# Dellintel98/smart-nanogrid-gym

Hardware: AMD Instinct MI355X
Metric: env-steps/sec (whole node) at N=65,536 envs × 10 chargers, 24-step day (higher is better)
Workload: dtype f64; 1 GPU; 65536 envs/GPU x 10 chargers x 24-step day, b-pv bounded sparse 1h, GPU-RNG reset + 24 fused steps per bench step (hipGraph); envs_per_gpu=65536, chargers=10, step_unit=one simulated day of every env, days_per_graph_replay=11, parallelism=env-sharded x1

## Files before the change

smart-nanogrid-gym_amd/csrc/sng_dev_env.h:

```cpp
#pragma once

namespace sng {

__device__ __forceinline__ void write_obs_header(float *o, const Params &p, const double *irr, const double *pn,
                                                 double ratio, const double *fpv, const double *fpr) {
    int k = 0;
    if (p.pv) o[k++] = (float)((irr[0] * ratio) * fpv[0]);
    o[k++] = (float)(pn[0] * fpr[0]);
    if (p.pv) {
#pragma unroll
        for (int j = 1; j <= 3; ++j) o[k++] = (float)((irr[j] * ratio) * fpv[j]);
    }
#pragma unroll
    for (int j = 1; j <= 3; ++j) o[k++] = (float)(pn[j] * fpr[j]);
}

__device__ __forceinline__ void write_obs_header_station(float *o, const double *irr, const float *pnf, double ratio) {
    o[0] = (float)(irr[0] * ratio);
    o[1] = pnf[0];
#pragma unroll
    for (int j = 1; j <= 3; ++j) {
        o[1 + j] = (float)(irr[j] * ratio);
        o[4 + j] = pnf[j];
    }
}

__device__ __forceinline__ uint32_t mix32(uint32_t x) {
    x ^= x >> 17;
    x *= 0xed5ad4bbu;
    x ^= x >> 11;
    x *= 0xac4c1b51u;
    x ^= x >> 15;
    x *= 0x31848babu;
    x ^= x >> 14;
    return x;
}

__device__ __forceinline__ uint32_t stream_key(uint64_t seed, uint64_t ge, uint32_t lane, uint64_t day) {
    const uint32_t k0 = mix32((uint32_t)seed ^ mix32((uint32_t)(seed >> 32) + (uint32_t)day * 0x9e3779b9u));
    const uint32_t k1 = mix32(k0 ^ (uint32_t)ge);
    return mix32(k1 ^ ((uint32_t)(ge >> 32) * 0x85ebca6bu + lane * 0xc2b2ae35u + 0x27d4eb2fu));
}

constexpr uint32_t kDomainPV = 0x50560000u;
constexpr uint32_t kDomainPrice = 0x50520000u;

__device__ __forceinline__ double profile_factor_key(uint32_t key, int k, double sigma) {
    if (sigma == 0.0) return 1.0;
    const uint32_t h = mix32(key + (uint32_t)k * 0x9e3779b9u);
    const double z = (double)h * 0x1.0p-31 - 1.0;
    return 1.0 + sigma * z;
}
__device__ __forceinline__ double profile_factor(uint64_t env_seed, uint32_t domain, uint64_t day, int k,
                                                 double sigma) {
    return profile_factor_key(stream_key(env_seed, 0, domain, day), k, sigma);
}
__device__ __forceinline__ v2u profile_keys(const DeviceState &s, uint32_t el8) {
    return __builtin_bit_cast(v2u, bld(reinterpret_cast<const uint64_t *>(s.prof_key), el8));
}
__device__ __forceinline__ void expand_profile_factors(const Params &p, v2u kk, int t, double *fpv, double *fpr) {
#pragma unroll
    for (int j = 0; j < 4; ++j) {
        fpv[j] = profile_factor_key(kk.x, t + j, p.pv_noise);
        fpr[j] = profile_factor_key(kk.y, t + j, p.price_noise);
    }
}
__device__ __forceinline__ void profile_factors(const Params &p, const DeviceState &s, uint32_t el8, int t,
                                                double *fpv, double *fpr) {
    expand_profile_factors(p, profile_keys(s, el8), t, fpv, fpr);
}

enum { CST_IRR = 0, CST_PN = 4, CST_PV = 8, CST_PRICE = 9, CST_COUNT = 10 };
__host__ __device__ inline double step_constant(const Tables *tb, int t, int i) {
    return i < CST_PN ? tb->irr_norm[t + i]
                      : i < CST_PV ? tb->price_norm[t + i - CST_PN] : i == CST_PV ? tb->pv_power[t] : tb->price[t];
}

__device__ __forceinline__ double step_constant_scalar(const Tables *tb, int t, int i) {
    typedef const __attribute__((address_space(4))) double *ConstF64;
    const double *q = i < CST_PN ? &tb->irr_norm[t + i]
                                 : i < CST_PV ? &tb->price_norm[t + i - CST_PN] : i == CST_PV ? &tb->pv_power[t] : &tb->price[t];
    return *(ConstF64)(uintptr_t)q;
}

template <bool PK = false>
__device__ __forceinline__ float departure_obs(uint32_t w) {
    const float d = PK ? (float)(w >> P_DEP_SHIFT) : (float)((w >> W_DEP_SHIFT) & 0xffu);
    constexpr float r24 = 1.0f / 24.0f;
    const float q = d * r24;
    return __builtin_fmaf(__builtin_fmaf(-q, 24.0f, d), r24, q);
}

__device__ __forceinline__ double div_by_cap(double x, double c, double r) {
    const double q = x * r;
    return __builtin_fma(__builtin_fmin(__builtin_fma(-q, c, x), q), r, q);
}

__device__ __forceinline__ double recip_cap(double c) {
    const double r0 = __builtin_amdgcn_rcp(c);
    return __builtin_fma(r0, __builtin_fma(-c, r0, 1.0), r0);
}

struct ChargerResult {
    double pw;
    double q;
    double soc;
    uint32_t nx;
    uint32_t fl;
};

template <bool FAST, bool NONNEG = false, bool PK = false>
__device__ __forceinline__ ChargerResult charger_step(const Params &p, uint32_t w, double aux, double run, double req,
                                                      float a, int t, double rcap) {
    ChargerResult o;
    SNG_DIAG_CHARGER(o, aux, run, a);
    const double margin = 0.05 * req;
    const double d = (req - run) * 10;
    const bool insufficient = (t > 0) && (w & W_PEN) && (run < req - margin);
    o.q = insufficient ? d * d : 0.0;

    const bool occ = (w & W_OCC) != 0;
    const double prev = (occ && !(w & W_STATIC)) ? run : aux;
    const uint32_t capi = cap_field<PK>(w);
    const double cap = (double)capi;
    const bool idle = (a == 0.0f);
    const bool chg = (a > 0.0f);
    static_assert(FAST || !NONNEG, "the NONNEG form is the wide kernel's: NumPy-2 promotion");
    double pc, calc, calc_dis;
    float pf = 0.0f;
    if (!FAST && p.legacy) {
        pc = ((double)a * p.ev_power) * p.ev_eff;
        calc = calc_dis = prev + (pc * p.dt) / cap;
    } else {
        pf = __fmul_rn(__fmul_rn(a, p.ev_power_f), p.ev_eff_f);
        const float pdt = __fmul_rn(pf, p.dt_f);
        pc = (double)pf;
        const double mag = div_by_cap(NONNEG ? (double)pdt : __builtin_fabs((double)pdt), cap, rcap);
        calc = prev + mag;
        calc_dis = prev - mag;
    }
    if constexpr (NONNEG) {
        const bool moved = occ && chg && p.bounded;
        o.soc = moved ? ((1.0 < calc) ? 1.0 : calc) : prev;
        o.pw = (double)(moved ? pf : 0.0f);
        o.nx = (!occ && chg) ? 1u : 0u;
        o.fl = (occ && chg && !p.bounded) ? (uint32_t)SNG_FLAG_CHARGING_MODE : 0u;
        return o;
    }
    double pw_dis = pc;
    if (FAST) {
        pw_dis = !(calc_dis < 0.0) ? -((prev * cap) * p.rdt) : pc;
    } else if (occ && !idle && !chg && !(calc_dis < 0.0)) {
        const double x = prev * cap;
        pw_dis = -(p.dt_pow2 ? x * p.rdt : x / p.dt);
    }
    const double soc_chg = (1.0 < calc) ? 1.0 : calc;
    const double soc_dis = (calc_dis > 0.0) ? calc_dis : 0.0;
    const bool moved = occ && !idle && p.bounded;
    o.soc = moved ? (chg ? soc_chg : soc_dis) : prev;
    o.pw = moved ? (chg ? pc : pw_dis) : 0.0;
    o.nx = (!occ && !idle) ? 1u : 0u;
    o.fl = (occ && !idle && !p.bounded) ? (uint32_t)SNG_FLAG_CHARGING_MODE : 0u;
    return o;
}

template <bool PK>
struct ChargerVisit {
    ChargerResult r;
    double soc;
    uint32_t w_dep;
    __device__ __forceinline__ float obs_soc() const { return (float)r.soc; }
    __device__ __forceinline__ float obs_dep() const { return departure_obs<PK>(w_dep); }
};
template <bool FAST, bool NONNEG, bool PK, bool TABLE = false>
__device__ __forceinline__ ChargerVisit<PK> visit_charger(const Params &p, uint32_t w, const double &aux, double run,
                                                          double req, float a, int t, const double *rcp_table = nullptr) {
    const uint32_t capi = cap_field<PK>(w);
    const bool occ = (w & W_OCC) != 0;
    ChargerVisit<PK> v{charger_step<FAST, NONNEG, PK>(p, PK ? (w & ~W_STATIC) : w, PK ? 0.0 : aux, run, req, a, t,
                                                      TABLE ? rcp_table[capi] : recip_cap((double)capi)),
                       0.0, (PK && !occ) ? 0u : w};
    v.soc = (PK && !occ) ? (double)rec_soc(w) : v.r.soc;
    return v;
}

struct BessStep {
    double bess, pen_b, bpow, bcalc, pw, dp;
    bool moved, chg;
    uint32_t fl;
};
template <bool STORE = true>
__device__ __forceinline__ BessStep bess_step(const Params &p, const DeviceState &s, uint32_t el8, int t, double bess,
                                              float bess_action) {
    BessStep b{bess, 0.0, 0.0, 0.0, 0.0, 0.0, false, false, 0u};
    if (!p.bess) return b;
    if (t == 0) bst(s.bess0, el8, bess);
    const double ba = (double)bess_action;
    b.chg = ba > 0.0;
    b.pw = (ba * (b.chg ? p.bess_pmax_ch : p.bess_pmax_dis)) * (b.chg ? p.bess_eff_ch : p.bess_eff_dis);
    const double calc = bess + (b.pw * p.dt) / p.bess_cap;
    const double empty = bess * p.bess_cap;
    b.dp = !(calc >= 0.0) ? -(p.dt_pow2 ? empty * p.rdt : empty / p.dt) : b.pw;
    if (ba == 0.0) {
        b.bpow = 0.0;
        b.bcalc = 0.0;
    } else if (!p.bounded) {
        b.fl |= SNG_FLAG_CHARGING_MODE;
    } else {
        b.moved = true;
        b.bcalc = b.pw;
        b.bess = b.chg ? ((1.0 < calc) ? 1.0 : calc) : ((calc > 0.0) ? calc : 0.0);
        b.bpow = b.chg ? b.pw : b.dp;
    }
    if (b.bess < p.bess_dod) {
        const double d = (p.bess_dod - b.bess) * 10;
        b.pen_b = d * d;
    } else if (!(b.bess <= 1.0)) {
        b.fl |= SNG_FLAG_BESS_SOC_ABOVE_1;
    }
    if constexpr (STORE) bst<kNT>(s.bess, el8, b.bess);
    return b;
}

static_assert((SNG_FLAG_NEGATIVE_DEMAND | SNG_FLAG_CHARGING_MODE | SNG_FLAG_BESS_SOC_ABOVE_1 | SNG_FLAG_V2X_BREAKPOINT) == 0xfu,
              "env_tail ORs the flag summary bit by bit: bits 0-3");
template <bool DIAG, bool PRE = false, bool KEEP = false>
__device__ __forceinline__ void env_tail(const Params &p, const DeviceState &s, const InfoPtrs &info, int64_t e0, uint32_t lo, uint32_t el1, uint32_t el8,
                                         int t, double ratio, double bess, float bess_action, double p_ch,
                                         double p_dis, double pen_v, double nonexist, uint32_t fl, float *o_row,
                                         const double *cst, const double *fpv, const double *fpr, double ret_prev,
                                         double bess0, double *__restrict__ reward, uint8_t *__restrict__ done,
                                         const BessStep *pre = nullptr, double *ret_keep = nullptr) {
    const double solar = p.pv ? (cst[CST_PV] * ratio) * fpv[0] : 0.0;
    const double demand = p_ch + p_dis;
    if (demand < 0.0) fl |= p.v2x ? SNG_FLAG_V2X_BREAKPOINT : SNG_FLAG_NEGATIVE_DEMAND;
    double rem = demand - solar;

    if (p.bess && t == 0) bess0 = bess;
    const BessStep b = PRE ? *pre : bess_step(p, s, el8, t, bess, bess_action);
    fl |= b.fl;
    if (b.moved) rem = b.chg ? -((-rem) - b.pw) : rem + b.dp;
    const double pen_b = b.pen_b, bpow = b.bpow, bcalc = b.bcalc;
    bess = b.bess;

    const double grid = rem;
    const double energy = grid * p.dt;
    const double price = cst[CST_PRICE] * fpr[0];
    const double cost = (energy < 0.0) ? (energy * p.sell_coef) * price : energy * price;
    const double tot_pen = p.bat_pen_w * pen_b + pen_v;
// ... 53 lines not shown
```

smart-nanogrid-gym_amd/csrc/sng_kernels.hip:

```cpp
#include <hip/hip_ext.h>
#include <hip/hip_runtime.h>
#include <stdint.h>

#include <initializer_list>
#include <type_traits>

#include "sng.h"
#include "sng_graph_form.h"
#include "sng_launch.h"
#include "sng_layout.h"
#include "sng_step_plan.h"

#include "sng_dev_util.h"
#include "sng_dev_sums.h"
#include "sng_exact_sum.h"
#include "sng_dev_env.h"
#include "sng_step_lean.h"
#include "sng_step_wide.h"
#include "sng_step_day.h"
#include "sng_step_general.h"
#include "sng_generate.h"
#include "sng_policy.h"
#include "sng_policy_net.h"
#include "sng_ppo.h"
// ... 15 lines not shown

template <class Kernel, class... Args>
static hipError_t launch_kernel(Kernel kern, dim3 grid, dim3 block, size_t lds, hipStream_t stream,
                                hipEvent_t ev_start, hipEvent_t ev_stop, Args... args) {
    if (ev_start && ev_stop)
        hipExtLaunchKernelGGL(kern, grid, block, (uint32_t)lds, stream, ev_start, ev_stop, 0u, args...);
    else
        hipLaunchKernelGGL(kern, grid, block, lds, stream, args...);
    return hipGetLastError();
}

hipError_t launch_probe_copy(const void *in, void *out, int64_t nr, int64_t nw, hipStream_t stream, hipEvent_t a,
                             hipEvent_t b) {
    const int64_t n = nr > nw ? nr : nw;
    const dim3 grid((unsigned)((n + 255) / 256)), block(256);
    return launch_kernel(probe_copy_kernel, grid, block, 0, stream, a, b, (const float4 *)in, (float4 *)out, nr, nw);
}

SNG_DIAG_SET_STAMPS

typedef void (*ConstStepKernel)(const float *, float *, double *, uint8_t *, int64_t, int, int, StepConst, Params,
                                DeviceState, InfoPtrs);
typedef void (*GeneralStepKernel)(Params, DeviceState, InfoPtrs, const float *, float *, double *, uint8_t *, int64_t,
                                  int, int);
struct StepLaunch {
    ConstStepKernel by_const = nullptr;
    GeneralStepKernel general = nullptr;
    dim3 grid, block;
    size_t lds = 0;
};

static dim3 blocks_for(int64_t E, int envs_per_block) { return dim3((unsigned)((E + envs_per_block - 1) / envs_per_block)); }

template <int NC>
static StepLaunch lean_launch(const StepPlan &pl, int64_t E) {
    static constexpr ConstStepKernel k[2][2] = {{step_lean_kernel<NC, false, false>, step_lean_kernel<NC, false, true>},
                                                {step_lean_kernel<NC, true, false>, step_lean_kernel<NC, true, true>}};
    return {k[pl.pk][pl.req], nullptr, blocks_for(E, kLeanBlock), dim3(kLeanBlock), LeanLds<NC>::BYTES};
}

template <int NC>
static StepLaunch wide_launch(const StepPlan &pl, int64_t E) {
    constexpr int L = kWideLanes;
    static constexpr ConstStepKernel k[2][2][2] = {
        {{step_wide_kernel<NC, L, false, false, false>, step_wide_kernel<NC, L, false, false, true>},
         {step_wide_kernel<NC, L, false, true, false>, step_wide_kernel<NC, L, false, true, true>}},
        {{step_wide_kernel<NC, L, true, false, false>, step_wide_kernel<NC, L, true, false, true>},
         {step_wide_kernel<NC, L, true, true, false>, step_wide_kernel<NC, L, true, true, true>}}};
    using Lay = WideLds<NC, L>;
    return {k[pl.pk][pl.req][pl.noise], nullptr, blocks_for(E, Lay::WENVS), dim3(kWave), Lay::BYTES};
}

template <int NC, int L>
static StepLaunch general_launch(const StepPlan &pl, const Params &p, int64_t E) {
    static constexpr GeneralStepKernel k[2][2][2] = {
        {{step_kernel<NC, L, false, false, false>, step_kernel<NC, L, false, false, true>},
         {step_kernel<NC, L, false, true, false>, step_kernel<NC, L, false, true, true>}},
        {{step_kernel<NC, L, true, false, false>, step_kernel<NC, L, true, false, true>},
         {step_kernel<NC, L, true, true, false>, step_kernel<NC, L, true, true, true>}}};
    using Lay = StepLds<NC, L>;
    return {nullptr, k[pl.diag][pl.fast][pl.pk], blocks_for(E, Lay::ENVS), dim3(Lay::BLOCK),
            Lay::bytes(p.act_dim, p.obs_dim)};
}

template <int NC>
static StepLaunch general_launch_lanes(const StepPlan &pl, const Params &p, int64_t E) {
    return pl.lanes == 4   ? general_launch<NC, 4>(pl, p, E)
           : pl.lanes == 2 ? general_launch<NC, 2>(pl, p, E)
                           : general_launch<NC, 1>(pl, p, E);
}

template <int... Ns, class F>
static bool with_size(int nc, F f) {
    return ((nc == Ns && (f(std::integral_constant<int, Ns>{}), true)) || ...);
}
template <class F>
static bool with_lean_size(int nc, F f) {
    return with_size<1, 2, 4, 8, 10, 16>(nc, f);
}

static StepLaunch step_launch(const StepPlan &pl, const Params &p, int64_t E) {
    StepLaunch l;
    switch (pl.family) {
        case STEP_LEAN: with_lean_size(pl.nc, [&](auto n) { l = lean_launch<decltype(n)::value>(pl, E); }); break;
        case STEP_WIDE: with_size<10, 50>(pl.nc, [&](auto n) { l = wide_launch<decltype(n)::value>(pl, E); }); break;
        case STEP_GENERAL:
            if (!with_size<0, 1>(pl.nc, [&](auto n) { l = general_launch<decltype(n)::value, 1>(pl, p, E); }))
                with_size<2, 4, 8, 10, 16, 50>(pl.nc, [&](auto n) { l = general_launch_lanes<decltype(n)::value>(pl, p, E); });
            break;
    }
    return l;
}

hipError_t launch_step(const Params &p, const DeviceState &s, const InfoPtrs &info, const Tables &tab,
                       const float *act, float *obs, double *reward, uint8_t *done, int64_t E, int t, int vec_io,
                       hipStream_t stream, hipEvent_t ev_start, hipEvent_t ev_stop) {
    const StepLaunch l = step_launch(step_plan(p, info_diag(info)), p, E);
    if (l.general)
        return launch_kernel(l.general, l.grid, l.block, l.lds, stream, ev_start, ev_stop, p, s, info, act, obs, reward,
                             done, E, t, vec_io);
    if (!l.by_const) return hipErrorInvalidDeviceFunction;
    StepConst k;
    for (int i = 0; i < CST_COUNT; ++i) k.v[i] = step_constant(&tab, t, i);
    return launch_kernel(l.by_const, l.grid, l.block, l.lds, stream, ev_start, ev_stop, act, obs, reward, done, E, t,
                         vec_io, k, p, s, info);
}

typedef void (*DayKernel)(const float *, float *, double *, uint8_t *, int64_t, int, int, int, Params, DeviceState,
                          InfoPtrs);
typedef void (*DayLeanKernel)(const float *, float *, double *, uint8_t *, int64_t, int, int, int, int64_t, int64_t,
                              Params, DeviceState, InfoPtrs);
template <int NC>
static StepLaunch day_launch(const StepPlan &pl, int64_t E, DayKernel &kern) {
    constexpr int L = kWideLanes;
    static constexpr DayKernel k[2][2] = {{day_wide_kernel<NC, L, false, false>, day_wide_kernel<NC, L, false, true>},
                                          {day_wide_kernel<NC, L, true, false>, day_wide_kernel<NC, L, true, true>}};
    using Lay = WideLds<NC, L>;
    kern = k[pl.req][pl.noise];
    return {nullptr, nullptr, blocks_for(E, Lay::WENVS), dim3(kWave), Lay::BYTES};
}
template <int NC, bool PK, bool REQ>
static DayLeanKernel day_lean_entry() {
    if constexpr (day_lean_compiled(NC, PK, REQ)) return day_lean_kernel<NC, PK, REQ>;
    else return nullptr;
}
template <int NC>
static StepLaunch day_lean_launch(const StepPlan &pl, int64_t E, DayLeanKernel &kern) {
    const DayLeanKernel k[2][2] = {{day_lean_entry<NC, false, false>(), day_lean_entry<NC, false, true>()},
                                   {day_lean_entry<NC, true, false>(), day_lean_entry<NC, true, true>()}};
    kern = k[pl.pk][pl.req];
    return {nullptr, nullptr, blocks_for(E, kLeanBlock), dim3(kLeanBlock), LeanLds<NC>::BYTES};
}

hipError_t launch_day(DayNode node, const Params &p, const DeviceState &s, const InfoPtrs &info, const float *act,
                      float *obs, double *reward, uint8_t *done, int64_t E, int t0, int nt, int vec_io, hipStream_t stream,
                      int64_t obs_step, int64_t out_step) {
    const StepPlan pl = step_plan(p, info_diag(info));
    const DayFamily fam = day_kernel_of(pl, obs_step != 0 || out_step != 0);
    const bool wide = node == DAY_KERNEL_WIDE || node == DAY_KERNEL_STATION;
    if (fam == DAY_NONE || (fam == DAY_WIDE) != wide || (fam == DAY_LEAN) != (node == DAY_KERNEL_LEAN) ||
        (node == DAY_KERNEL_STATION && !day_station_fixed(pl, p)))
        return hipErrorNotSupported;
    if (t0 < 0 || nt < 1 || t0 + nt > p.T) return hipErrorInvalidValue;
    if (wide) {
        DayKernel kern = nullptr;
        const StepLaunch l = day_launch<10>(pl, E, kern);
        if (node == DAY_KERNEL_STATION) {
            static_assert(kDayStationN == 10 && kWideLanes == 2, "day_launch<10>'s geometry");
            const DayStationArgs a{act, obs, reward, done, E, t0, nt, vec_io, p.bump_day, p.dt_f, p.ev_power_f, p.ev_eff_f,
                                   p.dt, p.rdt, p.bess_cap, p.bess_pmax_ch, p.bess_pmax_dis, p.bess_eff_ch,
                                   p.bess_eff_dis, p.bess_dod, p.grid_w, p.bat_pen_w, p.sell_coef, s.soc, s.bess,
                                   s.bess0, s.ratio, s.pen0, s.aux, s.flags, s.episode, s.tables, info.flags,
                                   info.flag_any, info.episode_return};
            return launch_kernel(day_station_kernel<kDayStationN, kWideLanes>, l.grid, l.block,
                                 l.lds + sizeof(StationRows), stream, nullptr, nullptr, a);
        }
        return launch_kernel(kern, l.grid, l.block, l.lds, stream, nullptr, nullptr, act, obs, reward, done, E, t0, nt,
                             vec_io, p, s, info);
    }
    DayLeanKernel kern = nullptr;
    StepLaunch l;
    with_lean_size(pl.nc, [&](auto n) { l = day_lean_launch<decltype(n)::value>(pl, E, kern); });
    if (!kern) return hipErrorInvalidDeviceFunction;
    if (obs_step % 4 != 0) vec_io = 0;
    return launch_kernel(kern, l.grid, l.block, l.lds, stream, nullptr, nullptr, act, obs, reward, done, E, t0, nt,
                         vec_io, obs_step, out_step, p, s, info);
}

hipError_t launch_observe0(const Params &p, const DeviceState &s, float *obs, double *ep_return, int64_t E,
                           int vec_io, hipStream_t stream, int mode, int64_t replay, const RefStreams *ps, int py) {
    const RefStreams no_streams{nullptr, nullptr};
    const RefStreams &pss = (py && ps) ? *ps : no_streams;
    if (!ps) py = 0;
    const bool big = (size_t)round4(256 * p.obs_dim) * 4 <= 64 * 1024;
    const int envs = big ? 256 : kWave;
    auto kern = big ? (p.packed ? observe0_kernel<256, true> : observe0_kernel<256, false>)
                    : (p.packed ? observe0_kernel<kWave, true> : observe0_kernel<kWave, false>);
    return launch_kernel(kern, blocks_for(E, envs), dim3(envs), (size_t)round4(envs * p.obs_dim) * 4, stream, nullptr,
                         nullptr, p, s, obs, ep_return, E, vec_io, mode, replay, pss, py);
}

hipError_t launch_generate(const Params &p, const DeviceState &s, uint64_t seed, int64_t E, int i4, int i10, int i1,
                           float *obs, double *ep_return, int vec_io, hipStream_t stream, hipEvent_t ev_start,
                           hipEvent_t ev_stop, int day_delta, size_t min_lds) {
    const size_t veh = generate_lds_bytes(p.req_enabled != 0), tile = (size_t)round4(kObsEnvs * p.obs_dim) * 4;
    const bool fused = generator_fused(p);
    if (!fused && (day_delta != 0 || !obs)) return hipErrorInvalidValue;
    const dim3 grid((unsigned)((E + kGenBlock - 1) / kGenBlock), (unsigned)(gen_rows(p.n) + (fused ? kObsBlocks : 0))),
        block(kGenBlock);
    size_t lds = (fused && obs && tile > veh) ? tile : veh;
    if (min_lds > lds) lds = min_lds;
    const bool req = p.req_enabled != 0;
    auto kern = p.T == 24 ? (req ? generate_kernel<24, true> : generate_kernel<24, false>)
                : (p.T == 96 && !req) ? generate_kernel<96, false>
                : (req ? generate_kernel<0, true> : generate_kernel<0, false>);
    if (fused && ev_start && ev_stop)
        return launch_kernel(kern, grid, block, lds, stream, ev_start, ev_stop, p, s, seed, E, i4, i10, i1, obs,
                             ep_return, vec_io, day_delta);
    if (ev_start) (void)hipEventRecord(ev_start, stream);
    hipError_t e = launch_kernel(kern, grid, block, lds, stream, nullptr, nullptr, p, s, seed, E, i4, i10, i1, obs,
                                 ep_return, vec_io, day_delta);
    if (!fused) {
        if (e == hipSuccess) e = launch_profiles(p, s, E, stream);
        if (e == hipSuccess) e = launch_observe0(p, s, obs, ep_return, E, vec_io, stream, OBS0_DEVICE, -1);
    }
    if (e == hipSuccess && ev_stop) e = hipEventRecord(ev_stop, stream);
    return e;
}

}

#include "sng_ref_day.h"

namespace sng {

static int ref_day2_envs(int64_t E) {
    return E >= 65536 ? 64 : E >= 16384 ? 32 : E >= 4096 ? 16 : 8;
}

template <int TT, bool REQ, int ENVS>
static void launch_ref_day2_envs(dim3 grid, dim3 block, size_t lds, hipStream_t stream, const Params &p,
                                 const DeviceState &s, const RefStreams &rs, int64_t E, int i4, int i10, int i1) {
    static const hipError_t set = hipFuncSetAttribute(reinterpret_cast<const void *>(ref_day2_kernel<TT, REQ, ENVS>),
                                                      hipFuncAttributeMaxDynamicSharedMemorySize,
                                                      (int)ref_day2_lds_bytes(REQ, ENVS));
    (void)set;
    hipLaunchKernelGGL((ref_day2_kernel<TT, REQ, ENVS>), grid, block, lds, stream, p, s, rs, E, i4, i10, i1);
}

template <int TT, bool REQ>
static void launch_ref_day2(const Params &p, const DeviceState &s, const RefStreams &rs, int64_t E, int i4, int i10,
                            int i1, hipStream_t stream) {
    const int envs = ref_day2_envs(E);
    const int64_t per = (int64_t)envs * kRefGroups;
    const dim3 grid((unsigned)((E + per - 1) / per)), block(kRefBlock);
    const size_t lds = ref_day2_lds_bytes(REQ, envs);
    with_size<8, 16, 32, 64>(envs, [&](auto n) {
        launch_ref_day2_envs<TT, REQ, decltype(n)::value>(grid, block, lds, stream, p, s, rs, E, i4, i10, i1);
    });
}

hipError_t launch_ref_seed(const RefStreams &rs, uint64_t seed0, int64_t E, hipStream_t stream) {
    hipLaunchKernelGGL(mt_seed_kernel, dim3((unsigned)((E + 255) / 256)), dim3(256), 0, stream, rs, seed0, E);
    return hipGetLastError();
}

hipError_t launch_mt_prepare(const RefStreams &rs, int64_t E, hipStream_t stream) {
    hipLaunchKernelGGL(mt_prepare_kernel, dim3((unsigned)((E + 3) / 4)), dim3(256), 0, stream, rs, E);
    return hipGetLastError();
}

hipError_t launch_ref_day(const Params &p, const DeviceState &s, const RefStreams &rs, int64_t E, int i4, int i10,
                          int i1, bool prepare, hipStream_t stream) {
    if (prepare) {
        hipError_t e = launch_mt_prepare(rs, E, stream);
        if (e != hipSuccess) return e;
    }
    const bool req = p.req_stream != 0;
    auto launch = p.T == 24 ? (req ? launch_ref_day2<24, true> : launch_ref_day2<24, false>)
                            : (req ? launch_ref_day2<0, true> : launch_ref_day2<0, false>);
    launch(p, s, rs, E, i4, i10, i1, stream);
    return hipGetLastError();
}

__global__ void bump_day_kernel(DeviceState s, uint64_t amount) {
    __hip_atomic_fetch_add(s.episode, amount, __ATOMIC_RELAXED, __HIP_MEMORY_SCOPE_AGENT);
}

hipError_t launch_bump_day(const DeviceState &s, hipStream_t stream, uint64_t amount) {
    hipLaunchKernelGGL(bump_day_kernel, dim3(1), dim3(1), 0, stream, s, amount);
    return hipGetLastError();
}

typedef void (*PolicyDayKernel)(const float *, PolicyImage, const float *, int64_t, int, const float *, float *, float *,
                                double *, uint8_t *, int64_t, int, int, int, int, int64_t, int64_t, int64_t, Params,
                                DeviceState, InfoPtrs);
template <int NC, bool PK, bool REQ>
static PolicyDayKernel policy_day_entry() {
    if constexpr (policy_day_compiled(NC, PK, REQ)) return day_lean_policy_kernel<NC, PK, REQ>;
    else return nullptr;
}
template <int NC>
static StepLaunch policy_day_launch(const StepPlan &pl, int64_t E, PolicyDayKernel &kern) {
    const PolicyDayKernel k[2][2] = {{policy_day_entry<NC, false, false>(), policy_day_entry<NC, false, true>()},
                                     {policy_day_entry<NC, true, false>(), policy_day_entry<NC, true, true>()}};
    kern = k[pl.pk][pl.req];
    return {nullptr, nullptr, blocks_for(E, kLeanBlock), dim3(kLeanBlock), PolicyDayLds<NC>::BYTES};
}

hipError_t launch_policy_day(const Params &p, const DeviceState &s, const InfoPtrs &info, const float *img,
                             const PolicyImage &m, const float *noise, const float *obs0, float *obs,
                             float *actions_out, double *reward, uint8_t *done, int64_t E, int vec_io,
                             hipStream_t stream, int64_t obs_step, int64_t out_step, int64_t act_step) {
    const StepPlan pl = step_plan(p, info_diag(info));
    if (m.O != p.obs_dim || m.A != p.act_dim) return hipErrorInvalidValue;
    PolicyDayKernel kern = nullptr;
    StepLaunch l;
    if (pl.family == STEP_LEAN)
        with_lean_size(pl.nc, [&](auto n) { l = policy_day_launch<decltype(n)::value>(pl, E, kern); });
    if (!kern) return hipErrorInvalidDeviceFunction;
    const int64_t noise_step = noise ? E * (int64_t)p.act_dim : 0;
    if (obs_step % 4 != 0 || !aligned16(obs0) || !aligned16(noise) || noise_step % 4 != 0) vec_io = 0;
    const int vec_act = (aligned16(actions_out) && act_step % 4 == 0) ? 1 : 0;
    return launch_kernel(kern, l.grid, l.block, l.lds, stream, nullptr, nullptr, img, m, noise ? noise : actions_out,
                         noise_step, noise ? 1 : 0, obs0, obs, actions_out, reward, done, E, 0, p.T, vec_io, vec_act,
                         obs_step, out_step, act_step, p, s, info);
}

// ... 208 lines not shown
```

smart-nanogrid-gym_amd/csrc/sng_step_day.h:

```cpp
#pragma once

namespace sng {

template <int NC, int L, bool REQ, bool NOISE>
__global__ __launch_bounds__(kWave) __attribute__((amdgpu_waves_per_eu(L, L))) void
day_wide_kernel(const float *__restrict__ act, float *__restrict__ obs, double *__restrict__ reward,
                uint8_t *__restrict__ done, int64_t E, int t0, int nt, int vec_io, Params p, DeviceState s,
                InfoPtrs info) {
    using Grp = WideGroup<NC, L, true, REQ, NOISE>;
    using Lay = WideLds<NC, L>;
    extern __shared__ __attribute__((aligned(16))) float lds[];
    const int lane = threadIdx.x;
    float *s_obs = lds + Lay::ACT;
    Grp g;
    const int64_t e0 = (int64_t)blockIdx.x * Grp::WENVS;
    const size_t block = (size_t)E * (size_t)p.act_dim;
    g.template issue<true, false>(e0, act, E, t0, vec_io, p, s, info, lane);
    v2u keys = {0u, 0u};
    if constexpr (NOISE) keys = profile_keys(s, g.el8);
#pragma unroll
    for (int j = 0; j < 4; ++j) g.fpv[j] = g.fpr[j] = 1.0;
    g.issue_step_inputs(act, E, t0, vec_io, p, s, lane);
    wave_vmem_drain();
    constexpr unsigned kPinned = (REQ || NOISE) ? 0x303u : 0x3ffu;
    const int t1 = t0 + nt;
#pragma unroll 1
    for (int t = t0; t < t1; ++t) {
        g.stamp_step_top();
        g.take_step_inputs();
        g.day_tile.commit(lds, lane);
        wave_lds_fence();
        if constexpr (NOISE) expand_profile_factors(p, keys, t, g.fpv, g.fpr);
        if (t + 1 < t1)
            g.issue_step_inputs(act + (size_t)(t + 1 - t0) * block, E, t + 1, vec_io, p, s, lane);
        StepConst k;
#pragma unroll
        for (int i = 0; i < CST_COUNT; ++i) {
            k.v[i] = step_constant_scalar(s.tables, t, i);
            if (kPinned & (1u << i)) asm("" : "+v"(k.v[i]));
        }
        g.template run<true>(lds, s_obs, obs, reward, done, E, t, vec_io, k, p, s, info, lane);
        wave_lds_fence();
    }
    SNG_WSTAMP_FLUSH(g.stamp_, 5);
    g.store_state(E, p, s, info, lane);
    bump_day_counter<true>(p, s, t0);
}

struct DayStationArgs {
    const float *act;
    float *obs;
    double *reward;
    uint8_t *done;
    int64_t E;
    int32_t t0, nt, vec_io, bump_day;
    float dt_f, ev_power_f, ev_eff_f;
    double dt, rdt;
    double bess_cap, bess_pmax_ch, bess_pmax_dis, bess_eff_ch, bess_eff_dis, bess_dod;
    double grid_w, bat_pen_w, sell_coef;
    double *soc, *bess, *bess0, *ratio, *pen0, *rec;
    uint32_t *flags;
    uint64_t *episode;
    const Tables *tables;
    uint32_t *info_flags, *flag_any;
    double *episode_return;
};
struct StationRows {
    static constexpr int N = kDayStationT + 3;
    double irr[N];
    double env[N][2];
    float pnf[N + 1];
};
template <int NC, int L>
__global__ __launch_bounds__(kWave) __attribute__((amdgpu_waves_per_eu(L, L))) void day_station_kernel(DayStationArgs a) {
    Params p{};
    p.n = NC;
    p.T = kDayStationT;
    p.act_dim = NC + 1;
    p.obs_dim = 2 * NC + 9;
    p.pv = p.bess = p.bounded = p.dt_pow2 = p.packed = 1;
    p.lanes = 1;
    p.bump_day = a.bump_day;
    p.dt = a.dt;
    p.rdt = a.rdt;
    p.dt_f = a.dt_f;
    p.ev_power_f = a.ev_power_f;
    p.ev_eff_f = a.ev_eff_f;
    p.bess_cap = a.bess_cap;
    p.bess_pmax_ch = a.bess_pmax_ch;
    p.bess_pmax_dis = a.bess_pmax_dis;
    p.bess_eff_ch = a.bess_eff_ch;
    p.bess_eff_dis = a.bess_eff_dis;
    p.bess_dod = a.bess_dod;
    p.grid_w = a.grid_w;
    p.bat_pen_w = a.bat_pen_w;
    p.sell_coef = a.sell_coef;
    DeviceState s{};
    s.soc = a.soc;
    s.bess = a.bess;
    s.bess0 = a.bess0;
    s.ratio = a.ratio;
    s.pen0 = a.pen0;
    s.aux = a.rec;
    s.flags = a.flags;
    s.episode = a.episode;
    s.tables = a.tables;
    InfoPtrs info{};
    info.flags = a.info_flags;
    info.flag_any = a.flag_any;
    info.episode_return = a.episode_return;
    using Grp = WideGroup<NC, L, true, false, false>;
    using Lay = WideLds<NC, L>;
    extern __shared__ __attribute__((aligned(16))) float lds[];
    const int lane = threadIdx.x;
    float *s_obs = lds + Lay::ACT;
    Grp g;
    const int64_t E = a.E;
    const int t0 = a.t0, vec_io = a.vec_io;
    const float *__restrict__ act = a.act;
    float *__restrict__ obs = a.obs;
    double *__restrict__ reward = a.reward;
    uint8_t *__restrict__ done = a.done;
    const int64_t e0 = (int64_t)blockIdx.x * Grp::WENVS;
    const size_t block = (size_t)E * (size_t)p.act_dim, plane = (size_t)NC * (size_t)E;
    const float *act_t = act;
    const uint16_t *rec_t = packed_records(s) + (size_t)(t0 + 1) * plane;
    StationRows *rows = reinterpret_cast<StationRows *>(lds + Lay::ACT + Lay::OBS);
    const int row_i = lane < StationRows::N ? lane : StationRows::N - 1;
    const Tables *tb = a.tables;
    const double row_irr = tb->irr_norm[row_i], row_pn = tb->price_norm[row_i], row_pv = tb->pv_power[row_i],
                 row_price = tb->price[row_i];
    g.template issue<true, false>(e0, act, E, t0, vec_io, p, s, info, lane);
#pragma unroll
    for (int j = 0; j < 4; ++j) g.fpv[j] = g.fpr[j] = 1.0;
    g.issue_step_inputs_at(act_t, rec_t, E, vec_io, lane);
    wave_vmem_drain();
    rows->irr[row_i] = row_irr;
    rows->pnf[row_i] = (float)row_pn;
    rows->env[row_i][0] = row_pv;
    rows->env[row_i][1] = row_price;
    wave_lds_fence();
    const int t1 = t0 + a.nt;
#pragma unroll 1
    for (int t = t0; t < t1; ++t) {
        g.stamp_step_top();
        StepConst k;
        StationStep st;
#pragma unroll
        for (int j = 0; j < 4; ++j) {
            k.v[CST_IRR + j] = rows->irr[t + j];
            k.v[CST_PN + j] = 0.0;
            st.pnf[j] = rows->pnf[t + j];
        }
        k.v[CST_PV] = rows->env[t][0];
        k.v[CST_PRICE] = rows->env[t][1];
        st.rec_t = rec_t;
        g.take_step_inputs();
        g.day_tile.commit(lds, lane);
        wave_lds_fence();
        act_t += block;
        rec_t += plane;
        if (t + 1 < t1) g.issue_step_inputs_at(act_t, rec_t, E, vec_io, lane);
        g.template run<true, true>(lds, s_obs, obs, reward, done, E, t, vec_io, k, p, s, info, lane, &st);
        wave_lds_fence();
    }
    SNG_WSTAMP_FLUSH(g.stamp_, 5);
    g.store_state(E, p, s, info, lane);
    bump_day_counter<true>(p, s, t0);
}

constexpr int kDayLeanWaves = 1;
template <int NC, bool PK, bool REQ>
__global__ __launch_bounds__(kLeanBlock) __attribute__((amdgpu_waves_per_eu(kDayLeanWaves))) void
day_lean_kernel(const float *__restrict__ act, float *__restrict__ obs, double *__restrict__ reward,
                uint8_t *__restrict__ done, int64_t E, int t0, int nt, int vec_io, int64_t obs_step, int64_t out_step,
                Params p, DeviceState s, InfoPtrs info) {
    static_assert(kLeanBlock == kWave, "one wavefront per workgroup");
    extern __shared__ __attribute__((aligned(16))) float lds[];
    const int lane = threadIdx.x;
    const LeanTiles<NC> tl(lds, 0);
    LeanGroup<NC, PK, REQ> g;
    const size_t block = (size_t)E * (size_t)p.act_dim;
    g.template issue<true, false>((int64_t)blockIdx.x * kLeanBlock, act, E, t0, vec_io, p, s, info, lane);
    g.issue_step_inputs(act, E, t0, vec_io, p, s, lane);
    const int t1 = t0 + nt;
#pragma unroll 1
    for (int t = t0; t < t1; ++t) {
        g.take_step_inputs(p);
        g.act_tile.commit(tl.s_act, lane);
        wave_lds_fence();
        const StepConst k = g.kn;
        if (t + 1 < t1)
            g.issue_step_inputs(act + (size_t)(t + 1 - t0) * block, E, t + 1, vec_io, p, s, lane);
        g.template run<true>(tl.s_act, tl.s_obs, tl.s_pos, tl.s_neg, obs, reward, done, E, t, vec_io, k, p, s, info, lane);
        wave_lds_fence();
        obs += obs_step;
        reward += out_step;
        done += out_step;
    }
    g.store_state(E, p, s, info);
    bump_day_counter<PK>(p, s, t0);
}

}
```

smart-nanogrid-gym_amd/csrc/sng_step_wide.h:

```cpp
#pragma once

namespace sng {


struct StationStep {
    float pnf[4];
    const uint16_t *rec_t;
};

template <int NC, int L>
struct WideLds {
    static constexpr int WENVS = kWave / L;
    static constexpr int A = NC + 1;
    static constexpr int O = 2 * NC + 9;
    static constexpr int ACT = round4(WENVS * A), OBS = round4(WENVS * O);
    static constexpr size_t BYTES = (size_t)(ACT + OBS) * 4;
};

template <int K>
__device__ __forceinline__ uint32_t from_part(uint32_t x) {
    constexpr int ctrl = K | (K << 2) | ((K + 2) << 4) | ((K + 2) << 6);
    return (uint32_t)__builtin_amdgcn_mov_dpp((int)x, ctrl, 0xF, 0xF, false);
}
template <int K>
__device__ __forceinline__ double from_part(double x) {
    const uint64_t b = __builtin_bit_cast(uint64_t, x);
    const uint64_t lo = from_part<K>((uint32_t)b), hi = from_part<K>((uint32_t)(b >> 32));
    return __builtin_bit_cast(double, lo | (hi << 32));
}

template <int NC, int L, bool PK, bool REQ, bool NOISE>
struct WideGroup {
    using Lay = WideLds<NC, L>;
    static_assert(L == 2 && NC % 8 == 2, "two lanes per env, each with whole charger pairs and record quads");
    static constexpr int WENVS = Lay::WENVS, H = (NC - 2) / 2, CPL = H + 1;
    static constexpr int KT = (Lay::A * WENVS + 4 * kWave - 1) / (4 * kWave);
    static constexpr bool kNonneg = NC <= 16;
    static __device__ __forceinline__ int charger(int part, int j) { return j < H ? part * H + j : NC - 2 + part; }
    int64_t e0;
    int nw;
    bool live;
    uint32_t el1, el4, el8, row4, row4_last, soc_a, soc_b, rec_a, rec_b;
    TileStage<KT, kWave> act_tile;
    double ratio, bess_l, pen0_l, ret_l;
    double fpv[4], fpr[4];
    uint32_t w[CPL];
    double aux[PK ? 1 : CPL], run_[CPL], req[REQ ? CPL : 1];
    SNG_WSTAMP_DECL;
    __device__ __forceinline__ void stamp_step_top() { SNG_WSTAMP(0); }

    static __device__ __forceinline__ uint32_t r4_of(int j, int64_t E) {
        return (uint32_t)(j < H ? j : NC - 2) * (uint32_t)E * 4u;
    }
    __device__ __forceinline__ uint32_t row_of(int j) const { return j < H ? row4 : row4_last; }
    __device__ __forceinline__ void place(int64_t e0_, int64_t E, int lane) {
        const int le = lane / L, part = lane % L;
        e0 = e0_;
        nw = (E - e0) < WENVS ? (int)(E - e0) : WENVS;
        live = le < nw;
        const int64_t el = live ? e0 + le : E - 1;
        el1 = (uint32_t)el;
        el4 = el1 * 4u;
        el8 = el1 * 8u;
        row4 = el4 + (uint32_t)(part * H) * (uint32_t)E * 4u;
        row4_last = el4 + (uint32_t)part * (uint32_t)E * 4u;
        soc_a = 2u * el8 + (uint32_t)(part * H) * (uint32_t)E * 8u;
        soc_b = 2u * el8 + (uint32_t)part * 8u;
        rec_a = el1 * 8u + (uint32_t)(part * H) * (uint32_t)E * 2u;
        rec_b = el1 * 4u + (uint32_t)part * 2u;
    }
    __device__ __forceinline__ void issue_soc(int j, int64_t E, const DeviceState &s) {
        if (j < H && (j & 1)) bld2(s.soc, soc_a, (uint32_t)(j - 1) * (uint32_t)E * 8u, run_[j - 1], run_[j]);
        if (j == H) run_[j] = bld(s.soc, soc_b, (uint32_t)(NC - 2) * (uint32_t)E * 8u);
    }
    __device__ __forceinline__ void store_soc(int j, int64_t E, const DeviceState &s, const double *v) {
        if (j < H && (j & 1)) bst2<kNT>(s.soc, soc_a, v[j - 1], v[j], (uint32_t)(j - 1) * (uint32_t)E * 8u);
        if (j == H) bst<kNT>(s.soc, soc_b, v[j], (uint32_t)(NC - 2) * (uint32_t)E * 8u);
    }
    __device__ __forceinline__ void store_state_soc(int64_t E, const DeviceState &s) {
        if (live) {
#pragma unroll
            for (int j = 0; j < CPL; ++j) store_soc(j, E, s, run_);
        }
    }
    __device__ __forceinline__ void store_state(int64_t E, const Params &p, const DeviceState &s, const InfoPtrs &info,
                                                int lane) {
        store_state_soc(E, s);
        if (live && lane % L == 0) {
            if (p.bess) bst<kNT>(s.bess, el8, bess_l);
            if (info.episode_return) bst<kNT>(info.episode_return, el8, ret_l);
        }
    }
    template <bool STATE = true, bool STEP = true>
    __device__ __forceinline__ void issue(int64_t e0_, const float *act, int64_t E, int t, int vec_io, const Params &p,
                                          const DeviceState &s, const InfoPtrs &info, int lane) {
        SNG_WSTAMP(0);
        place(e0_, E, lane);
        [[maybe_unused]] const size_t plane = (size_t)t * NC * (size_t)E;
        [[maybe_unused]] const uint16_t *rec_t = packed_records(s) + plane + (size_t)NC * (size_t)E;
        [[maybe_unused]] const int Ad = p.act_dim;
        if constexpr (STEP) act_tile.issue(act + e0 * Ad, nw * Ad, vec_io != 0, lane);
        if constexpr (STATE) {
            ratio = bld(s.ratio, el8);
            bess_l = bld(p.bess ? s.bess : s.ratio, el8);
        }
        if constexpr (STEP) {
#pragma unroll
            for (int j = 0; j < 4; ++j) fpv[j] = fpr[j] = 1.0;
            if constexpr (NOISE) profile_factors(p, s, el8, t, fpv, fpr);
        }
#pragma unroll
        for (int j = 0; j < CPL; ++j) {
            const uint32_t v4 = row_of(j), r4 = r4_of(j, E), v8 = 2u * v4, r8 = 2u * r4;
            if constexpr (STEP) {
                if (PK) {
                    if (j < H && (j & 3) == 0)
                        unpack_quad(bld(reinterpret_cast<const uint64_t *>(rec_t), rec_a, (uint32_t)j * (uint32_t)E * 2u),
                                    w + j);
                    if (j == H) w[j] = bld16(rec_t, rec_b, (uint32_t)(NC - 2) * (uint32_t)E * 2u);
                } else {
                    w[j] = bld(s.word + plane, v4, r4);
                    aux[PK ? 0 : j] = bld(s.aux + plane, v8, r8);
                }
            }
            if constexpr (STATE) issue_soc(j, E, s);
            if constexpr (STEP)
                if (REQ) req[REQ ? j : 0] = bld(s.req + plane, v8, r8);
        }
        if constexpr (STATE) {
            pen0_l = bld(t == 0 ? s.pen0 : s.ratio, el8);
            ret_l = bld(info.episode_return ? info.episode_return : s.ratio, el8);
        }
    }
    static constexpr int NQ = H / 4;
    TileStage<KT, kWave, true> day_tile;
    uint64_t rq[NQ];
    uint32_t rl;
    double reqn[REQ ? CPL : 1];
    __device__ __forceinline__ void issue_step_inputs(const float *act, int64_t E, int t, int vec_io, const Params &p,
                                                      const DeviceState &s, int lane) {
        static_assert(PK, "the day kernel steps packed days");
        const size_t plane = (size_t)t * NC * (size_t)E;
        const uint16_t *rec_t = packed_records(s) + plane + (size_t)NC * (size_t)E;
        day_tile.issue(act + e0 * p.act_dim, nw * p.act_dim, vec_io != 0, lane);
#pragma unroll
        for (int q = 0; q < NQ; ++q)
            rq[q] = bld(reinterpret_cast<const uint64_t *>(rec_t), rec_a, (uint32_t)(4 * q) * (uint32_t)E * 2u);
        rl = bld16(rec_t, rec_b, (uint32_t)(NC - 2) * (uint32_t)E * 2u);
        if constexpr (REQ) {
#pragma unroll
            for (int j = 0; j < CPL; ++j) reqn[j] = bld(s.req + plane, 2u * row_of(j), 2u * r4_of(j, E));
        }
    }
    __device__ __forceinline__ void issue_step_inputs_at(const float *act_t, const uint16_t *rec_t, int64_t E, int vec_io,
                                                         int lane) {
        static_assert(PK && !REQ, "the default station's packed days");
        day_tile.issue(act_t + e0 * Lay::A, nw * Lay::A, vec_io != 0, lane);
#pragma unroll
        for (int q = 0; q < NQ; ++q)
            rq[q] = bld(reinterpret_cast<const uint64_t *>(rec_t), rec_a, (uint32_t)(4 * q) * (uint32_t)E * 2u);
        rl = bld16(rec_t, rec_b, (uint32_t)(NC - 2) * (uint32_t)E * 2u);
    }
    __device__ __forceinline__ void take_step_inputs() {
#pragma unroll
        for (int q = 0; q < NQ; ++q) unpack_quad(rq[q], w + 4 * q);
        w[H] = rl;
        if constexpr (REQ) {
#pragma unroll
            for (int j = 0; j < CPL; ++j) req[j] = reqn[j];
        }
    }
    __device__ __forceinline__ double req_of(int j, const Params &p) const {
        return REQ ? req[REQ ? j : 0] : req_default(p);
    }

    template <bool KEEP = false, bool STATION = false>
    __device__ __forceinline__ void run(const float *s_act, float *s_obs, float *obs, double *reward, uint8_t *done,
                                        int64_t E, int t, int vec_io, const StepConst &k, const Params &p,
                                        const DeviceState &s, const InfoPtrs &info, int lane,
                                        const StationStep *st = nullptr) {
        static_assert(!STATION || (KEEP && PK && !REQ && !NOISE && kNonneg), "the default station's day kernel");
        SNG_WSTAMP(1);
        const int Ad = p.act_dim, O = p.obs_dim;
        const int le = lane / L, part = lane % L;
        const bool leader = part == 0;
        const size_t plane = (size_t)t * NC * (size_t)E;
        const uint16_t *rec_t = packed_records(s) + plane + (size_t)NC * (size_t)E;
        if constexpr (STATION) rec_t = st->rec_t;
        const float *a_row = s_act + le * Ad;
        float *o_row = s_obs + le * O;
        float av[CPL];
        uint32_t amax_bits = 0u;
#pragma unroll
        for (int j = 0; j < CPL; ++j) {
            av[j] = a_row[charger(part, j)];
            amax_bits = __builtin_elementwise_max(amax_bits, __builtin_bit_cast(uint32_t, av[j]));
        }
        const bool not_nonneg = amax_bits > 0x7f800000u;
        const float bess_action = p.bess ? a_row[NC] : 0.0f;
        const int k_soc = p.pv ? 8 : 4;
        BessStep bs{};
        if (live && leader) {
            if constexpr (STATION) write_obs_header_station(o_row, k.v + CST_IRR, st->pnf, ratio);
            else write_obs_header(o_row, p, k.v + CST_IRR, k.v + CST_PN, ratio, fpv, fpr);
            bs = bess_step<!KEEP>(p, s, el8, t, p.bess ? bess_l : 0.0, bess_action);
            if (p.bess) o_row[O - 1] = (float)bs.bess;
        }

        double pen_v = 0.0, p_ch = 0.0, p_dis = 0.0;
        uint32_t n_nonexist = 0, fl = 0;
        if (__builtin_amdgcn_ballot_w64(live && not_nonneg) == 0) {
            double seq_pos = 0.0, pmin = __builtin_inf();
            int n_pos = 0;
            uint32_t bmax = kExactSumBmax0, bmin = kExactSumBmin0;
            double qv[CPL], sv[CPL];
            if (live) {
#pragma unroll
                for (int j = 0; j < CPL; ++j) {
                    const int c = charger(part, j);
                    const uint32_t capi = cap_field<PK>(w[j]);
                    const bool occ = (w[j] & W_OCC) != 0;
                    const ChargerResult r = charger_step<true, kNonneg, PK>(p, PK ? (w[j] & ~W_STATIC) : w[j],
                                                                           PK ? 0.0 : aux[PK ? 0 : j], run_[j], req_of(j, p),
                                                                           av[j], t, recip_cap((double)capi));
                    sv[j] = (PK && !occ) ? (double)rec_soc(w[j]) : r.soc;
                    if constexpr (KEEP) run_[j] = sv[j];
                    else store_soc(j, E, s, sv);
                    o_row[k_soc + c] = (float)r.soc;
                    o_row[k_soc + NC + c] = departure_obs<PK>((PK && !occ) ? 0u : w[j]);
                    n_nonexist += r.nx;
                    fl |= r.fl;
                    qv[j] = r.q;
                    if (j < H) pen_v += r.q;
                    if constexpr (STATION) {
                        seq_pos += r.pw;
                        exact_sum_track(exact_sum_hi(r.pw), bmax, bmin);
                    } else {
                        const bool ip = r.pw > 0.0;
                        seq_pos += r.pw;
                        n_pos += ip ? 1 : 0;
                        pmin = __builtin_fmin(pmin, ip ? r.pw : __builtin_inf());
                    }
                    __builtin_amdgcn_sched_barrier(0);
                }
            }
            const double seq_own = seq_pos, pmin_own = pmin;
            const int n_own = n_pos;
            const uint32_t nx_own = n_nonexist, fl_own = fl;
            int with_pos = n_own > 0 ? 1 : 0;
            const uint32_t bmax_own = bmax, bmin_own = bmin;
            auto gather = [&] {
                if constexpr (STATION) {
                    bmax = __builtin_elementwise_max(bmax, from_part<1>(bmax_own));
                    bmin = __builtin_elementwise_min(bmin, from_part<1>(bmin_own));
                    seq_pos += from_part<1>(seq_own);
                } else {
                    const int nk = (int)from_part<1>((uint32_t)n_own);
                    with_pos += nk > 0 ? 1 : 0;
                    n_pos += nk;
                    seq_pos += from_part<1>(seq_own);
                    pmin = __builtin_fmin(pmin, from_part<1>(pmin_own));
                }
                n_nonexist += from_part<1>(nx_own);
                fl |= from_part<1>(fl_own);
#pragma unroll
                for (int j = 0; j < H; ++j) {
                    const double qk = from_part<1>(qv[j]);
                    pen_v = (STATION || leader) ? pen_v + qk : pen_v;
                }
            };
            gather();
            {
                const double qk = from_part<1>(qv[H]);
                pen_v = (STATION || leader) ? (pen_v + qv[H]) + qk : pen_v;
            }
            const bool split = with_pos > 1;
            p_ch = seq_pos;
            bool pos_slow;
            if constexpr (STATION) pos_slow = live && leader && exact_sum_rebuild(bmax, bmin);
            else pos_slow = live && leader && (n_pos >= 8 || split) && !(seq_pos <= pmin * 0x1.0p28);
            if (__builtin_amdgcn_ballot_w64(pos_slow)) {
                if (pos_slow) {
                    PairwiseSum pos;
                    pos.init();
#pragma unroll 1
                    for (int c = 0; c < NC; ++c) {
                        const RecOff ro = rec_off(c, NC, E, el1);
                        const uint32_t wc = PK ? bld16(rec_t, ro.v, ro.s)
                                               : bld(s.word + plane, el4, (uint32_t)c * (uint32_t)E * 4u);
                        const float a = a_row[c];
                        const double pc = charging_power(p, a);
                        if ((wc & W_OCC) && p.bounded && a > 0.0f && pc > 0.0) pos.push(pc);
                    }
                    p_ch = pos.result();
                }
            }
        } else {
            PairwiseSum pos, neg;
            pos.init();
            neg.init();
            if constexpr (KEEP) {
                store_state_soc(E, s);
                wave_mem_fence();
            }
            if (live && leader) {
#pragma unroll 1
                for (int c = 0; c < NC; ++c) {
                    const uint32_t r4 = (uint32_t)c * (uint32_t)E * 4u, r8 = 2u * r4;
                    const SocOff so = soc_off(c, NC, E, el8);
                    const RecOff ro = rec_off(c, NC, E, el1);
                    const uint32_t wc = PK ? bld16(rec_t, ro.v, ro.s) : bld(s.word + plane, el4, r4);
                    const double auxc = PK ? 0.0 : bld(s.aux + plane, el8, r8);
                    const double runc = bld(s.soc, so.v, so.s);
                    const double reqc = REQ ? bld(s.req + plane, el8, r8) : req_default(p);
                    const ChargerVisit<PK> v = visit_charger<true, false, PK>(p, wc, auxc, runc, reqc, a_row[c], t);
                    const ChargerResult &r = v.r;
                    bst<kNT>(s.soc, so.v, v.soc, so.s);
                    o_row[k_soc + c] = v.obs_soc();
                    o_row[k_soc + NC + c] = v.obs_dep();
                    n_nonexist += r.nx;
                    fl |= r.fl;
                    pen_v += r.q;
                    if (r.pw > 0.0) pos.push(r.pw);
                    if (r.pw < 0.0) neg.push(r.pw);
                }
            }
            p_ch = pos.result();
            p_dis = neg.result();
            if constexpr (KEEP) {
                wave_mem_fence();
#pragma unroll
                for (int j = 0; j < CPL; ++j) issue_soc(j, E, s);
                wave_vmem_drain();
            }
        }
        SNG_WSTAMP(2);
        if constexpr (KEEP) wave_vmem_drain();
        if (live && leader) {
            pen_v += (t == 0) ? pen0_l : 0.0;
            env_tail<false, true, KEEP>(p, s, info, e0, (uint32_t)le, el1, el8, t, ratio, p.bess ? bess_l : 0.0,
                                        bess_action, p_ch, p_dis, pen_v, 100.0 * (double)n_nonexist, fl, o_row, k.v, fpv,
                                        fpr, info.episode_return ? ret_l : 0.0, 0.0, reward, done, &bs, &ret_l);
            if constexpr (KEEP) bess_l = bs.bess;
        }
        SNG_WSTAMP(3);
        wave_lds_fence();
        copy_out<kWave>(obs + e0 * O, s_obs, nw * O, vec_io != 0, lane);
        SNG_WSTAMP(4);
    }
};

template <int NC, int L, bool PK, bool REQ, bool NOISE>
__global__ __launch_bounds__(kWave) __attribute__((amdgpu_waves_per_eu(L, L))) void
step_wide_kernel(const float *__restrict__ act, float *__restrict__ obs, double *__restrict__ reward,
                 uint8_t *__restrict__ done, int64_t E, int t, int vec_io, StepConst k, Params p, DeviceState s,
                 InfoPtrs info) {
    using Grp = WideGroup<NC, L, PK, REQ, NOISE>;
    using Lay = WideLds<NC, L>;
    extern __shared__ __attribute__((aligned(16))) float lds[];
    const int lane = threadIdx.x;
    float *s_obs = lds + Lay::ACT;
    Grp g;
    const int64_t e0 = (int64_t)blockIdx.x * Grp::WENVS;
    g.issue(e0, act, E, t, vec_io, p, s, info, lane);
    g.act_tile.commit(lds, lane);
    wave_lds_fence();
    g.run(lds, s_obs, obs, reward, done, E, t, vec_io, k, p, s, info, lane);
    SNG_WSTAMP_FLUSH(g.stamp_, 5);
    bump_day_counter<PK>(p, s, t);
}

}
```

Before: 19.97 billion env-steps/s.

## Table charger reciprocals in LDS and restructure station kernel LDS layout

The station day kernel now precomputes a 128-entry table of per-capacity reciprocals, loads it from the tables into LDS once, and looks it up per charger, with the next lookup issued one charger ahead. This replaces the rcp/FMA refinement sequence in the charger loop. The LDS layout drops the separate action tile: observations start at offset 0, the rows and reciprocal table follow, and the rare slow paths read actions straight from global memory. PV and price constants are now read by pointer from the LDS rows late in the step instead of being copied early. The change trades LDS reads and a new tb->recip dependency for less ALU work, and must match the old results bit for bit.

```diff
diff --git a/smart-nanogrid-gym_amd/csrc/sng_dev_env.h b/smart-nanogrid-gym_amd/csrc/sng_dev_env.h
--- a/smart-nanogrid-gym_amd/csrc/sng_dev_env.h
+++ b/smart-nanogrid-gym_amd/csrc/sng_dev_env.h
@@ -1,4 +1,6 @@
 #pragma once
+
+#include "sng_div_by_cap.h"
 
 namespace sng {
 
@@ -91,10 +93,6 @@
     return __builtin_fmaf(__builtin_fmaf(-q, 24.0f, d), r24, q);
 }
 
-__device__ __forceinline__ double div_by_cap(double x, double c, double r) {
-    const double q = x * r;
-    return __builtin_fma(__builtin_fmin(__builtin_fma(-q, c, x), q), r, q);
-}
 
 __device__ __forceinline__ double recip_cap(double c) {
     const double r0 = __builtin_amdgcn_rcp(c);
diff --git a/smart-nanogrid-gym_amd/csrc/sng_div_by_cap.h b/smart-nanogrid-gym_amd/csrc/sng_div_by_cap.h
--- /dev/null
+++ b/smart-nanogrid-gym_amd/csrc/sng_div_by_cap.h
@@ -0,0 +1,12 @@
+#pragma once
+
+#include "sng_layout.h"
+
+namespace sng {
+
+SNG_HD inline __attribute__((always_inline)) double div_by_cap(double x, double c, double r) {
+    const double q = x * r;
+    return __builtin_fma(__builtin_fmin(__builtin_fma(-q, c, x), q), r, q);
+}
+
+}
diff --git a/smart-nanogrid-gym_amd/csrc/sng_kernels.hip b/smart-nanogrid-gym_amd/csrc/sng_kernels.hip
--- a/smart-nanogrid-gym_amd/csrc/sng_kernels.hip
+++ b/smart-nanogrid-gym_amd/csrc/sng_kernels.hip
@@ -191,8 +191,10 @@
                                    p.bess_eff_dis, p.bess_dod, p.grid_w, p.bat_pen_w, p.sell_coef, s.soc, s.bess,
                                    s.bess0, s.ratio, s.pen0, s.aux, s.flags, s.episode, s.tables, info.flags,
                                    info.flag_any, info.episode_return};
-            return launch_kernel(day_station_kernel<kDayStationN, kWideLanes>, l.grid, l.block,
-                                 l.lds + sizeof(StationRows), stream, nullptr, nullptr, a);
+            using Sl = StationLds<WideLds<kDayStationN, kWideLanes>>;
+            static_assert(Sl::REQUEST == 5880, "the request tests/golden/graph_listings.json lists");
+            return launch_kernel(day_station_kernel<kDayStationN, kWideLanes>, l.grid, l.block, Sl::REQUEST, stream,
+                                 nullptr, nullptr, a);
         }
         return launch_kernel(kern, l.grid, l.block, l.lds, stream, nullptr, nullptr, act, obs, reward, done, E, t0, nt,
                              vec_io, p, s, info);
diff --git a/smart-nanogrid-gym_amd/csrc/sng_step_day.h b/smart-nanogrid-gym_amd/csrc/sng_step_day.h
--- a/smart-nanogrid-gym_amd/csrc/sng_step_day.h
+++ b/smart-nanogrid-gym_amd/csrc/sng_step_day.h
@@ -70,6 +70,16 @@
     double irr[N];
     double env[N][2];
     float pnf[N + 1];
+};
+template <class Lay>
+struct StationLds {
+    static constexpr size_t ROWS = (size_t)Lay::OBS * 4;
+    static constexpr size_t RCP = (ROWS + sizeof(StationRows) + 7) & ~(size_t)7;
+    static constexpr size_t END = RCP + (size_t)kStationRcp * 8;
+    static constexpr size_t REQUEST = Lay::BYTES + sizeof(StationRows);
+    static_assert(Lay::ACT <= Lay::OBS, "the actions tile fits the observation tile");
+    static_assert(ROWS % 8 == 0, "StationRows holds doubles");
+    static_assert(END <= REQUEST, "tiles, rows and the reciprocal table fit the wavefront's LDS request");
 };
 template <int NC, int L>
 __global__ __launch_bounds__(kWave) __attribute__((amdgpu_waves_per_eu(L, L))) void day_station_kernel(DayStationArgs a) {
@@ -113,7 +123,8 @@
     using Lay = WideLds<NC, L>;
     extern __shared__ __attribute__((aligned(16))) float lds[];
     const int lane = threadIdx.x;
-    float *s_obs = lds + Lay::ACT;
+    using Sl = StationLds<Lay>;
+    float *s_obs = lds;
     Grp g;
     const int64_t E = a.E;
     const int t0 = a.t0, vec_io = a.vec_io;
@@ -125,11 +136,15 @@
     const size_t block = (size_t)E * (size_t)p.act_dim, plane = (size_t)NC * (size_t)E;
     const float *act_t = act;
     const uint16_t *rec_t = packed_records(s) + (size_t)(t0 + 1) * plane;
-    StationRows *rows = reinterpret_cast<StationRows *>(lds + Lay::ACT + Lay::OBS);
+    char *const lds_b = reinterpret_cast<char *>(lds);
+    StationRows *rows = reinterpret_cast<StationRows *>(lds_b + Sl::ROWS);
+    double *rcp = reinterpret_cast<double *>(lds_b + Sl::RCP);
     const int row_i = lane < StationRows::N ? lane : StationRows::N - 1;
     const Tables *tb = a.tables;
     const double row_irr = tb->irr_norm[row_i], row_pn = tb->price_norm[row_i], row_pv = tb->pv_power[row_i],
                  row_price = tb->price[row_i];
+    static_assert(kStationRcp == 2 * kWave, "two entries a lane");
+    const double rcp_a = tb->recip[lane], rcp_b = tb->recip[lane + kWave];
     g.template issue<true, false>(e0, act, E, t0, vec_io, p, s, info, lane);
 #pragma unroll
     for (int j = 0; j < 4; ++j) g.fpv[j] = g.fpr[j] = 1.0;
@@ -139,6 +154,8 @@
     rows->pnf[row_i] = (float)row_pn;
     rows->env[row_i][0] = row_pv;
     rows->env[row_i][1] = row_price;
+    rcp[lane] = rcp_a;
+    rcp[lane + kWave] = rcp_b;
     wave_lds_fence();
     const int t1 = t0 + a.nt;
 #pragma unroll 1
@@ -152,14 +169,16 @@
             k.v[CST_PN + j] = 0.0;
             st.pnf[j] = rows->pnf[t + j];
         }
-        k.v[CST_PV] = rows->env[t][0];
-        k.v[CST_PRICE] = rows->env[t][1];
+        k.v[CST_PV] = k.v[CST_PRICE] = 0.0;
+        st.env = rows->env[t];
         st.rec_t = rec_t;
+        st.rcp = rcp;
         g.take_step_inputs();
         g.day_tile.commit(lds, lane);
         wave_lds_fence();
         act_t += block;
         rec_t += plane;
+        st.act_next = act_t;
         if (t + 1 < t1) g.issue_step_inputs_at(act_t, rec_t, E, vec_io, lane);
         g.template run<true, true>(lds, s_obs, obs, reward, done, E, t, vec_io, k, p, s, info, lane, &st);
         wave_lds_fence();
diff --git a/smart-nanogrid-gym_amd/csrc/sng_step_wide.h b/smart-nanogrid-gym_amd/csrc/sng_step_wide.h
--- a/smart-nanogrid-gym_amd/csrc/sng_step_wide.h
+++ b/smart-nanogrid-gym_amd/csrc/sng_step_wide.h
@@ -6,7 +6,12 @@
 struct StationStep {
     float pnf[4];
     const uint16_t *rec_t;
+    const float *act_next;
+    const double *env;
+    const double *rcp;
 };
+constexpr int kStationRcp = 128;
+static_assert(P_CAP_MASK == kStationRcp - 1, "one entry per value of the record's capacity field");
 
 template <int NC, int L>
 struct WideLds {
@@ -198,6 +203,8 @@
         }
         const bool not_nonneg = amax_bits > 0x7f800000u;
         const float bess_action = p.bess ? a_row[NC] : 0.0f;
+        [[maybe_unused]] const float *a_mem = nullptr;
+        if constexpr (STATION) a_mem = st->act_next - (size_t)E * (size_t)Lay::A + (size_t)el1 * (size_t)Lay::A;
         const int k_soc = p.pv ? 8 : 4;
         BessStep bs{};
         if (live && leader) {
@@ -214,15 +221,20 @@
             int n_pos = 0;
             uint32_t bmax = kExactSumBmax0, bmin = kExactSumBmin0;
             double qv[CPL], sv[CPL];
+            [[maybe_unused]] double rc_next = 0.0;
+            if constexpr (STATION) rc_next = st->rcp[cap_field<PK>(w[0])];
             if (live) {
 #pragma unroll
                 for (int j = 0; j < CPL; ++j) {
                     const int c = charger(part, j);
                     const uint32_t capi = cap_field<PK>(w[j]);
                     const bool occ = (w[j] & W_OCC) != 0;
+                    [[maybe_unused]] const double rc = rc_next;
+                    if constexpr (STATION)
+                        if (j + 1 < CPL) rc_next = st->rcp[cap_field<PK>(w[j + 1])];
                     const ChargerResult r = charger_step<true, kNonneg, PK>(p, PK ? (w[j] & ~W_STATIC) : w[j],
                                                                            PK ? 0.0 : aux[PK ? 0 : j], run_[j], req_of(j, p),
-                                                                           av[j], t, recip_cap((double)capi));
+                                                                           av[j], t, STATION ? rc : recip_cap((double)capi));
                     sv[j] = (PK && !occ) ? (double)rec_soc(w[j]) : r.soc;
                     if constexpr (KEEP) run_[j] = sv[j];
                     else store_soc(j, E, s, sv);
@@ -288,7 +300,7 @@
                         const RecOff ro = rec_off(c, NC, E, el1);
                         const uint32_t wc = PK ? bld16(rec_t, ro.v, ro.s)
                                                : bld(s.word + plane, el4, (uint32_t)c * (uint32_t)E * 4u);
-                        const float a = a_row[c];
+                        const float a = STATION ? a_mem[c] : a_row[c];
                         const double pc = charging_power(p, a);
                         if ((wc & W_OCC) && p.bounded && a > 0.0f && pc > 0.0) pos.push(pc);
                     }
@@ -313,7 +325,7 @@
                     const double auxc = PK ? 0.0 : bld(s.aux + plane, el8, r8);
                     const double runc = bld(s.soc, so.v, so.s);
                     const double reqc = REQ ? bld(s.req + plane, el8, r8) : req_default(p);
-                    const ChargerVisit<PK> v = visit_charger<true, false, PK>(p, wc, auxc, runc, reqc, a_row[c], t);
+                    const ChargerVisit<PK> v = visit_charger<true, false, PK>(p, wc, auxc, runc, reqc, STATION ? a_mem[c] : a_row[c], t);
                     const ChargerResult &r = v.r;
                     bst<kNT>(s.soc, so.v, v.soc, so.s);
                     o_row[k_soc + c] = v.obs_soc();
@@ -335,11 +347,18 @@
             }
         }
         SNG_WSTAMP(2);
+        [[maybe_unused]] StepConst kt;
+        const double *cst = k.v;
+        if constexpr (STATION) {
+            kt.v[CST_PV] = st->env[0];
+            kt.v[CST_PRICE] = st->env[1];
+            cst = kt.v;
+        }
         if constexpr (KEEP) wave_vmem_drain();
         if (live && leader) {
             pen_v += (t == 0) ? pen0_l : 0.0;
             env_tail<false, true, KEEP>(p, s, info, e0, (uint32_t)le, el1, el8, t, ratio, p.bess ? bess_l : 0.0,
-                                        bess_action, p_ch, p_dis, pen_v, 100.0 * (double)n_nonexist, fl, o_row, k.v, fpv,
+                                        bess_action, p_ch, p_dis, pen_v, 100.0 * (double)n_nonexist, fl, o_row, cst, fpv,
                                         fpr, info.episode_return ? ret_l : 0.0, 0.0, reward, done, &bs, &ret_l);
             if constexpr (KEEP) bess_l = bs.bess;
         }
```

After: 19.79 billion env-steps/s. About the same (-0.9%).
